# MicrobialDarkMatter/nanomotif

Measured on AMD Instinct MI355X. Metric: motif-sites scored/sec (1 Gbp synthetic metagenome), higher is better.
Workload: dtype u32 bit-planes / int64 counts

## Files before the change

nanomotif_amd/csrc/nmscan_device.h:

```cpp
#pragma once
#include "nmscan_internal.h"

namespace nmdetail {

__device__ __forceinline__ uint32_t alignbit(uint32_t hi, uint32_t lo, uint32_t sh) {
    return __builtin_amdgcn_alignbit(hi, lo, sh);
}

typedef const uint32_t __attribute__((address_space(4))) *cu32p;
typedef const uint8_t __attribute__((address_space(4))) *cu8p;

#ifndef NM_LIT_WAVES
#define NM_LIT_WAVES 4
#endif

template <int GN_, int GP_, bool COMPACT_, int NS_, bool LIT_, bool CF_, bool PC_ = false, bool CLS_ = false>
struct Variant {
    static constexpr int GN = GN_, GP = GP_, NS = NS_;
    static constexpr bool COMPACT = COMPACT_, LIT = LIT_, CF = CF_, PC = PC_;
    static constexpr bool CLS = CLS_;
    static_assert(!CLS || (GN == 1 && GP == 1 && COMPACT && NS == 1 && !LIT && !CF), "class planes: narrow compact heavy variants only");
    static constexpr int NW = T_WORDS + GN + GP;
    static constexpr int NP = LIT ? 4 : 8;
    static constexpr int NST = COMPACT ? 2 : 4;
    static constexpr int PDW = (GN + GP) * NP;
};

template <class K>
struct RawChunk {
    uint32_t h[K::NW], l[K::NW], v[K::NW];
    uint32_t s[K::NS][K::NST][T_WORDS];
    bool need_v;

    __device__ __forceinline__ void load(const Planes &seq, const StatePlanes (&stp)[K::NS], uint32_t chunk, int lane) {
        constexpr int GN = K::GN, GP = K::GP;
        need_v = ((cu8p)seq.needs_v)[chunk] != 0;
        const size_t base = (size_t)chunk * CHUNK_WORDS + (size_t)lane * T_WORDS;
#pragma unroll
        for (int j = 0; j < K::NS; ++j) {
            const uint32_t *src[4] = {K::COMPACT ? stp[j].M : stp[j].MP, K::COMPACT ? stp[j].U : stp[j].UP, stp[j].MM, stp[j].UM};
#pragma unroll
            for (int i = 0; i < K::NST; ++i) {
                const uint4 q = *reinterpret_cast<const uint4 *>(src[i] + base);
                s[j][i][0] = q.x; s[j][i][1] = q.y; s[j][i][2] = q.z; s[j][i][3] = q.w;
            }
        }
        const uint4 h4 = *reinterpret_cast<const uint4 *>(seq.H + base);
        const uint4 l4 = *reinterpret_cast<const uint4 *>(seq.L + base);
        h[GN + 0] = h4.x; h[GN + 1] = h4.y; h[GN + 2] = h4.z; h[GN + 3] = h4.w;
        l[GN + 0] = l4.x; l[GN + 1] = l4.y; l[GN + 2] = l4.z; l[GN + 3] = l4.w;
#pragma unroll
        for (int j = 0; j < GN; ++j) { h[j] = seq.H[base - GN + j]; l[j] = seq.L[base - GN + j]; }
#pragma unroll
        for (int j = 0; j < GP; ++j) { h[GN + T_WORDS + j] = seq.H[base + T_WORDS + j]; l[GN + T_WORDS + j] = seq.L[base + T_WORDS + j]; }
        if (need_v) {
            const uint4 v4 = *reinterpret_cast<const uint4 *>(seq.V + base);
            v[GN + 0] = v4.x; v[GN + 1] = v4.y; v[GN + 2] = v4.z; v[GN + 3] = v4.w;
#pragma unroll
            for (int j = 0; j < GN; ++j) v[j] = seq.V[base - GN + j];
#pragma unroll
            for (int j = 0; j < GP; ++j) v[GN + T_WORDS + j] = seq.V[base + T_WORDS + j];
        } else if constexpr (!K::CLS) {
#pragma unroll
            for (int j = 0; j < K::NW; ++j) v[j] = 0xFFFFFFFFu;
        }
    }
};

template <class K>
struct Tile {
    uint32_t w[K::NP][K::NW];

    __device__ __forceinline__ void expand(const RawChunk<K> &r) {
#pragma unroll
        for (int j = 0; j < K::NW; ++j) {
            const uint32_t hh = r.h[j], ll = r.l[j], vv = r.v[j];
            w[0][j] = vv & ~hh & ~ll;
            w[1][j] = vv & ~hh & ll;
            w[2][j] = vv & hh & ll;
            w[3][j] = vv & hh & ~ll;
            if (!K::LIT) {
                w[4][j] = vv & (hh | ll);
                w[5][j] = vv & (hh | ~ll);
                w[6][j] = vv & ~(hh & ll);
                w[7][j] = vv & (~hh | ll);
            }
        }
    }
};

template <class K>
__device__ __forceinline__ void eval_masks(const uint32_t (&m)[K::PDW], const Tile<K> &tile, uint32_t (&acc)[T_WORDS]) {
#pragma unroll
    for (int g = 0; g < K::GN + K::GP; ++g) {
#pragma unroll
        for (int p = 0; p < K::NP; ++p) {
            uint32_t mm = m[g * K::NP + p];
            while (mm) {
                const uint32_t r = __builtin_ctz(mm);
                mm &= mm - 1;
#pragma unroll
                for (int t = 0; t < T_WORDS; ++t) acc[t] &= alignbit(tile.w[p][t + g + 1], tile.w[p][t + g], r);
            }
        }
    }
}

constexpr int comp_plane(int p) { return (p & 4) | (3 - (p & 3)); }

template <class K>
struct JointWalk {
    uint32_t accf[T_WORDS], accr[T_WORDS];

    template <int G>
    static constexpr bool r0_possible() { return G > 0 && !(K::COMPACT && G == K::GN); }

    template <int I, bool R0 = false>
    __device__ __forceinline__ void and_in(const Tile<K> &tile, uint32_t r) {
        constexpr int G = I / K::NP, P = I % K::NP, CP = comp_plane(P), GR = R0 ? 2 * K::GN - G : 2 * K::GN - 1 - G;
        const uint32_t rr = R0 ? 0u : 32u - r;
#pragma unroll
        for (int t = 0; t < T_WORDS; ++t) accf[t] &= alignbit(tile.w[P][t + G + 1], tile.w[P][t + G], r);
#pragma unroll
        for (int t = 0; t < T_WORDS; ++t) accr[t] &= alignbit(tile.w[CP][t + GR + 1], tile.w[CP][t + GR], rr);
    }
    template <int I = 0>
    __device__ __forceinline__ void walk(const uint32_t (&m)[K::PDW], const Tile<K> &tile, const uint32_t (&bf)[T_WORDS],
                                         const uint32_t (&br)[T_WORDS]) {
        if constexpr (I == 0) {
#pragma unroll
            for (int t = 0; t < T_WORDS; ++t) { accf[t] = bf[t]; accr[t] = br[t]; }
        }
        if constexpr (I < K::PDW) {
            uint32_t mm = m[I];
            if (r0_possible<I / K::NP>() && (mm & 1u)) {
                mm &= ~1u;
                and_in<I, true>(tile, 0u);
            }
            while (mm) {
                const uint32_t r = __builtin_ctz(mm);
                mm &= mm - 1;
                and_in<I>(tile, r);
            }
            walk<I + 1>(m, tile, bf, br);
        }
    }
};

constexpr int CLS_PROG_DW = 32, CLS_SUMMARY_DW = 8, CLS_WORDS_DW = 9, CLS_BASE_DW = 29;
constexpr int cls_plane(int p) { return p < 4 ? p : p < 8 ? p - 4 : 4 + (p - 8) / 2; }
constexpr bool cls_neg(int p) { return p >= 4 && (p < 8 || ((p - 8) & 1)); }
constexpr int cls_mirror(int p) { return p < 4 ? 3 - p : p < 8 ? 11 - p : (p == 10 || p == 11) ? p : (p ^ 1); }
constexpr int cls_dword(int g, int p) { return p < 4 ? 4 * g + p : CLS_WORDS_DW + 10 * g + (p - 4); }
constexpr int cls_word_of_set(uint32_t set) {
    return set == 1 ? 0 : set == 2 ? 1 : set == 4 ? 2 : set == 8 ? 3 :
           set == 14 ? 4 : set == 13 ? 5 : set == 11 ? 6 : set == 7 ? 7 :
           set == 12 ? 8 : set == 3 ? 9 : set == 6 ? 10 : set == 9 ? 11 : set == 10 ? 12 : 13 ;
}

template <class K, bool BV>
struct ClassTile {
    static constexpr bool HAS_V = BV;
    static constexpr int VP = 6;
    uint32_t w[7][K::NW];

    __device__ __forceinline__ void expand(const RawChunk<K> &r) {
#pragma unroll
        for (int j = 0; j < K::NW; ++j) {
            const uint32_t hh = r.h[j], ll = r.l[j];
            w[0][j] = BV ? r.v[j] & ~(hh | ll) : ~(hh | ll);
            w[1][j] = ll & ~hh;
            w[2][j] = hh & ll;
            w[3][j] = hh & ~ll;
            w[4][j] = hh;
            w[5][j] = ll;
            w[6][j] = BV ? r.v[j] : hh ^ ll;
        }
    }
};

template <class K, class TileT>
struct ClassWalk {
    uint32_t accf[T_WORDS], accr[T_WORDS];

    template <int G, int P>
    __device__ __forceinline__ void and_one(const TileT &tile, uint32_t (&acc)[T_WORDS], uint32_t r) {
        constexpr int PL = cls_plane(P);
#pragma unroll
        for (int t = 0; t < T_WORDS; ++t) {
            uint32_t s;
            if constexpr (TileT::HAS_V && PL == 6) s = alignbit(tile.w[4][t + G + 1], tile.w[4][t + G], r) ^ alignbit(tile.w[5][t + G + 1], tile.w[5][t + G], r);
            else s = alignbit(tile.w[PL][t + G + 1], tile.w[PL][t + G], r);
            if constexpr (!cls_neg(P)) acc[t] &= s;
            else if constexpr (!TileT::HAS_V) acc[t] &= ~s;
            else acc[t] = acc[t] & ~s & alignbit(tile.w[TileT::VP][t + G + 1], tile.w[TileT::VP][t + G], r);
        }
    }
    template <int G, int P, bool R0 = false>
    __device__ __forceinline__ void and_in(const TileT &tile, uint32_t r) {
        constexpr int GR = R0 ? 2 * K::GN - G : 2 * K::GN - 1 - G;
        and_one<G, P>(tile, accf, r);
        and_one<GR, cls_mirror(P)>(tile, accr, R0 ? 0u : 32u - r);
    }
    template <int G, int P>
    __device__ __forceinline__ void word(uint32_t mm, const TileT &tile) {
        if (JointWalk<K>::template r0_possible<G>() && (mm & 1u)) {
            mm &= ~1u;
            and_in<G, P, true>(tile, 0u);
        }
        while (mm) {
            const uint32_t r = __builtin_ctz(mm);
            mm &= mm - 1;
            and_in<G, P>(tile, r);
        }
    }
    template <int Q>
    __device__ __forceinline__ void quad(const uint32_t (&m)[CLS_PROG_DW], const TileT &tile) {
        if (m[CLS_SUMMARY_DW] & (0xFu << (4 * Q))) {
            word<(4 * Q + 0) / 10, 4 + (4 * Q + 0) % 10>(m[CLS_WORDS_DW + 4 * Q + 0], tile);
            word<(4 * Q + 1) / 10, 4 + (4 * Q + 1) % 10>(m[CLS_WORDS_DW + 4 * Q + 1], tile);
            word<(4 * Q + 2) / 10, 4 + (4 * Q + 2) % 10>(m[CLS_WORDS_DW + 4 * Q + 2], tile);
            word<(4 * Q + 3) / 10, 4 + (4 * Q + 3) % 10>(m[CLS_WORDS_DW + 4 * Q + 3], tile);
        }
    }
    __device__ __forceinline__ void walk(const uint32_t (&m)[CLS_PROG_DW], const TileT &tile, const uint32_t (&)[T_WORDS],
                                         const uint32_t (&)[T_WORDS]) {
        const uint32_t cm = m[CLS_BASE_DW];
#pragma unroll
        for (int t = 0; t < T_WORDS; ++t) {
            accf[t] = (cm & tile.w[1][t + K::GN]) | (~cm & tile.w[0][t + K::GN]);
            accr[t] = (cm & tile.w[2][t + K::GN]) | (~cm & tile.w[3][t + K::GN]);
        }
        word<0, 0>(m[0], tile); word<0, 1>(m[1], tile); word<0, 2>(m[2], tile); word<0, 3>(m[3], tile);
        word<1, 0>(m[4], tile); word<1, 1>(m[5], tile); word<1, 2>(m[6], tile); word<1, 3>(m[7], tile);
        if (m[CLS_SUMMARY_DW]) {
            quad<0>(m, tile); quad<1>(m, tile); quad<2>(m, tile); quad<3>(m, tile); quad<4>(m, tile);
        }
    }
};

template <class K>
__device__ __forceinline__ void eval_strand(cu32p prog, const Tile<K> &tile, uint32_t (&acc)[T_WORDS]) {
    uint32_t m[K::PDW];
#pragma unroll
    for (int i = 0; i < K::PDW; ++i) m[i] = prog[i];
    eval_masks<K>(m, tile, acc);
}

inline uint32_t comp_mask(uint32_t m) { return ((m & 1) << 3) | ((m & 2) << 1) | ((m & 4) >> 1) | ((m & 8) >> 3); }

constexpr int PROG6_DW = 96;
inline int compile_program(const uint8_t *masks, uint32_t len, uint32_t modpos, uint32_t *prog, int *reach_class) {
    if (len == 0 || len > NM_MAX_MOTIF_LEN) return fail(NM_ERANGE, "motif length %u outside 1..%d", len, NM_MAX_MOTIF_LEN);
    if (modpos >= len) return fail(NM_EINVAL, "mod_position %u outside motif of length %u", modpos, len);
    memset(prog, 0, PROG6_DW * sizeof(uint32_t));
    bool any = false;
    *reach_class = 0;
    for (uint32_t j = 0; j < len; ++j) {
        const uint32_t m = masks[j] & 15u;
        if (m == 0) return fail(NM_EINVAL, "empty base set at motif position %u", j);
        if (m == 15u) continue;
        any = true;
        for (int strand = 0; strand < 2; ++strand) {
            const int d = strand == 0 ? (int)j - (int)modpos : (int)modpos - (int)j;
            const uint32_t set = strand == 0 ? m : comp_mask(m);
            const int gi = (d >> 5) + 3;
            const uint32_t r = (uint32_t)d & 31u;
            if (gi < 0 || gi > 5) return fail(NM_ERANGE, "offset %d from the modified base is outside [-96, 95]", d);
            *reach_class = std::max(*reach_class, gi == 0 || gi == 5 ? 2 : gi == 1 || gi == 4 ? 1 : 0);
            uint32_t *row = prog + strand * 48 + gi * 8;
            if (__builtin_popcount(set) == 1) {
                row[__builtin_ctz(set)] |= 1u << r;
            } else {
                uint32_t missing = (~set) & 15u;
                while (missing) {
                    row[4 + __builtin_ctz(missing)] |= 1u << r;
                    missing &= missing - 1;
                }
            }
        }
    }
    if (!any) return fail(NM_EINVAL, "motif has no specified position");
    return NM_OK;
}

inline void slice_program(const uint32_t *full, int G, uint32_t *out) {
    for (int strand = 0; strand < 2; ++strand)
        memcpy(out + strand * 2 * G * 8, full + strand * 48 + (3 - G) * 8, (size_t)2 * G * 8 * sizeof(uint32_t));
}

__device__ __forceinline__ void compile_one(uint32_t k, const CandRec *__restrict__ rec, const uint8_t *__restrict__ masks,
                                            uint32_t *__restrict__ programs, int wide, int np, int fold_modpos, uint32_t prog_slot = 0xFFFFFFFFu) {
    const int groups = 2 + 2 * wide, g0 = 1 - wide;
    const int pdw = 2 * groups * np;
    uint32_t *prog = programs + (size_t)(prog_slot == 0xFFFFFFFFu ? k : prog_slot) * pdw;
    for (int i = 0; i < pdw; ++i) prog[i] = 0;
    const CandRec c = rec[k];
    const uint8_t *m = masks + c.mask_off;
    for (int j = 0; j < c.len; ++j) {
        const uint32_t set_f = m[j] & 15u;
        if (set_f == 15u || (fold_modpos && j == c.modpos)) continue;
        for (int strand = 0; strand < 2; ++strand) {
            const int d = strand == 0 ? j - (int)c.modpos : (int)c.modpos - j;
            const uint32_t set = strand == 0 ? set_f
                                             : (((set_f & 1) << 3) | ((set_f & 2) << 1) | ((set_f & 4) >> 1) | ((set_f & 8) >> 3));
            const int g = (d >> 5) + 2 - g0;
            const uint32_t bit = 1u << ((uint32_t)d & 31u);
            uint32_t *row = prog + (strand * groups + g) * np;
            if (__popc(set) == 1) {
                row[__ffs(set) - 1] |= bit;
            } else {
                uint32_t missing = (~set) & 15u;
                while (missing) {
                    row[4 + __ffs(missing) - 1] |= bit;
                    missing &= missing - 1;
                }
            }
        }
    }
}

__device__ __forceinline__ void compile_one_classes(uint32_t k, const CandRec *__restrict__ rec, const uint8_t *__restrict__ masks,
                                                    uint32_t *__restrict__ programs, uint32_t c_slots) {
    uint32_t *prog = programs + (size_t)k * CLS_PROG_DW;
    for (int i = 0; i < CLS_PROG_DW; ++i) prog[i] = 0;
    const CandRec c = rec[k];
    const uint8_t *m = masks + c.mask_off;
    prog[CLS_BASE_DW] = ((c_slots >> c.slot) & 1u) ? 0xFFFFFFFFu : 0u;
    for (int j = 0; j < c.len; ++j) {
        const uint32_t set = m[j] & 15u;
        if (set == 15u || j == c.modpos) continue;
        const int d = j - (int)c.modpos;
        const int g = (d >> 5) + 1;
        if (g < 0 || g > 1) continue;
        const int p = cls_word_of_set(set);
        prog[cls_dword(g, p)] |= 1u << ((uint32_t)d & 31u);
        if (p >= 4) prog[CLS_SUMMARY_DW] |= 1u << (10 * g + p - 4);
    }
}

__device__ __forceinline__ void common_one(uint32_t g, uint4 *__restrict__ range, uint32_t *programs, uint32_t *commons, uint32_t pdw,
                                           uint32_t n_prog, uint32_t max_group) {
    uint4 r = range[g];
    r.z = 0xFFFFFFFFu;
    r.w = 0;
    if (r.y >= 2 && r.y <= max_group) {
        uint32_t *common = commons + (size_t)g * pdw;
        uint32_t any = 0;
        for (uint32_t i = 0; i < pdw; ++i) {
            uint32_t c = programs[(size_t)r.x * pdw + i];
            for (uint32_t k = 1; k < r.y; ++k) c &= programs[(size_t)(r.x + k) * pdw + i];
            common[i] = c;
            any |= c;
        }
        if (any) {
            bool single = true;
            const uint32_t sdw = pdw / 2;
            for (uint32_t k = 0; k < r.y; ++k) {
                uint32_t *prog = programs + (size_t)(r.x + k) * pdw;
                for (uint32_t i = 0; i < pdw; ++i) prog[i] &= ~common[i];
                for (uint32_t st = 0; st < 2; ++st) {
                    uint32_t bits = 0;
                    for (uint32_t i = 0; i < sdw; ++i) bits += __popc(prog[st * sdw + i]);
                    if (bits > 1) single = false;
                }
            }
            if (single) {
                for (uint32_t k = 0; k < r.y; ++k) {
                    uint32_t *prog = programs + (size_t)(r.x + k) * pdw;
                    uint32_t desc[2];
                    for (uint32_t st = 0; st < 2; ++st) {
                        desc[st] = sdw << 5;
                        for (uint32_t i = 0; i < sdw; ++i)
                            if (prog[st * sdw + i]) desc[st] = (i << 5) | (uint32_t)(__ffs(prog[st * sdw + i]) - 1);
                    }
                    prog[0] = desc[0];
                    prog[1] = desc[1];
                }
                r.w = 1;
            }
            r.z = n_prog + g;
        }
    }
    range[g] = r;
}


}

#ifdef NM_SCORE_KERNEL_SOURCE

namespace nmdetail {

struct ScoreArgs {
    Planes seq;
    StatePlanes st[NM_MAX_MOD_SLOTS];
    const uint4 *segments;
    uint32_t n_segments;
    uint32_t split_log2;
    uint32_t pieces_per_run, j_big, fine_log2;
    uint32_t n_bins;
    const uint4 *cand_range;
    const uint32_t *programs;
    const uint32_t *orig_index;
    unsigned long long *out;
    const uint32_t *chunk_rank;
    const uint64_t *row_base;
    uint32_t active_slot[NM_MAX_MOD_SLOTS];
    uint32_t slot_is_c[NM_MAX_MOD_SLOTS];
};

void launch_score_classes(const ScoreArgs &a, uint32_t gx, uint32_t gy, bool per_contig, hipStream_t s);

}

namespace {

using namespace nmdetail;

template <class K, int I = 0>
__device__ __forceinline__ void apply_single(uint32_t idx, uint32_t r, const Tile<K> &tile, const uint32_t (&base)[T_WORDS],
                                             uint32_t (&acc)[T_WORDS]) {
    if constexpr (I < K::PDW) {
        if (idx == I) {
            constexpr int g = I / K::NP, p = I % K::NP;
#pragma unroll
            for (int t = 0; t < T_WORDS; ++t) acc[t] = base[t] & alignbit(tile.w[p][t + g + 1], tile.w[p][t + g], r);
        } else {
            apply_single<K, I + 1>(idx, r, tile, base, acc);
        }
    } else {
#pragma unroll
        for (int t = 0; t < T_WORDS; ++t) acc[t] = base[t];
    }
}

template <class K>
__device__ __forceinline__ void emit_counts(const ScoreArgs &a, uint32_t n_mod, uint32_t n_non, uint32_t k0, uint32_t k,
                                            uint32_t *lds_acc, uint32_t lds_row0, int lane, uint32_t contig_rank) {
    if (K::PC) {
#pragma unroll
        for (int o = 32; o; o >>= 1) {
            n_mod += __shfl_xor(n_mod, o);
            n_non += __shfl_xor(n_non, o);
        }
        if (lane == 0 && (n_mod | n_non)) {
            unsigned long long *row = a.out + (a.row_base[k0 + k] + contig_rank) * 2;
            if (n_mod) atomicAdd(row, (unsigned long long)n_mod);
            if (n_non) atomicAdd(row + 1, (unsigned long long)n_non);
        }
        return;
    }
    atomicAdd(&lds_acc[((k * K::NS + lds_row0) * 2 + 0) * 64 + lane], n_mod);
    atomicAdd(&lds_acc[((k * K::NS + lds_row0) * 2 + 1) * 64 + lane], n_non);
}

template <class K, int CAN, class TileT>
__device__ __forceinline__ void score_heavy(const ScoreArgs &a, const TileT &tile, const uint32_t (&sw)[K::NST][T_WORDS],
                                            uint32_t k0, uint32_t nb, uint32_t *lds_acc, uint32_t lds_row0, int lane,
                                            uint32_t contig_rank) {
    constexpr int PF = CAN == 0 ? 0 : 1;
    constexpr int PR = CAN == 0 ? 3 : 2;
    uint32_t basef[T_WORDS], baser[T_WORDS];
#pragma unroll
    for (int t = 0; t < T_WORDS; ++t) {
        basef[t] = K::COMPACT ? tile.w[PF][t + K::GN] : 0xFFFFFFFFu;
        baser[t] = K::COMPACT ? tile.w[PR][t + K::GN] : 0xFFFFFFFFu;
    }
    constexpr int MDW = K::CLS ? CLS_PROG_DW : K::PDW;
    static_assert(!K::CLS || CLS_PROG_DW == 2 * K::PDW, "a class program takes the room of both halves of a plain one");
    std::conditional_t<K::CLS, ClassWalk<K, TileT>, JointWalk<K>> jw;
    for (uint32_t k = 0; k < nb; ++k) {
        cu32p prog = (cu32p)(a.programs + (size_t)(k0 + k) * (2 * K::PDW));
        uint32_t m[MDW];
        if constexpr (K::CLS) {
            typedef uint32_t u32x16 __attribute__((ext_vector_type(16)));
            typedef const u32x16 __attribute__((address_space(4))) *cu32x16p;
            const u32x16 lo = ((cu32x16p)prog)[0], hi = ((cu32x16p)prog)[1];
#pragma unroll
            for (int i = 0; i < 16; ++i) { m[i] = lo[i]; m[16 + i] = hi[i]; }
        } else {
#pragma unroll
            for (int i = 0; i < MDW; ++i) m[i] = prog[i];
        }
        jw.walk(m, tile, basef, baser);
        uint32_t n_mod = 0, n_non = 0;
#pragma unroll
        for (int t = 0; t < T_WORDS; ++t) {
            if (K::COMPACT) {
                const uint32_t sites = jw.accf[t] | jw.accr[t];
                n_mod += __popc(sites & sw[0][t]);
                n_non += __popc(sites & sw[1][t]);
            } else {
                n_mod += __popc(jw.accf[t] & sw[0][t]) + __popc(jw.accr[t] & sw[K::COMPACT ? 0 : 2][t]);
                n_non += __popc(jw.accf[t] & sw[1][t]) + __popc(jw.accr[t] & sw[K::COMPACT ? 1 : 3][t]);
            }
        }
        emit_counts<K>(a, n_mod, n_non, k0, k, lds_acc, lds_row0, lane, contig_rank);
    }
}

template <class K, int CAN, class TileT>
__device__ __forceinline__ void score_candidates(const ScoreArgs &a, const TileT &tile, const uint32_t (&sw)[K::NST][T_WORDS],
                                                 uint32_t k0, uint32_t nb, uint32_t common, bool siblings, uint32_t *lds_acc,
                                                 uint32_t lds_row0, int lane, uint32_t contig_rank = 0) {
    if constexpr (!K::CF) {
        score_heavy<K, CAN>(a, tile, sw, k0, nb, lds_acc, lds_row0, lane, contig_rank);
        return;
    } else {
    constexpr int PF = CAN == 0 ? 0 : 1;
    constexpr int PR = CAN == 0 ? 3 : 2;
    uint32_t basef[T_WORDS], baser[T_WORDS];
#pragma unroll
    for (int t = 0; t < T_WORDS; ++t) {
        basef[t] = K::COMPACT ? tile.w[PF][t + K::GN] : 0xFFFFFFFFu;
        baser[t] = K::COMPACT ? tile.w[PR][t + K::GN] : 0xFFFFFFFFu;
    }
    if (common != 0xFFFFFFFFu) {
        cu32p prog = (cu32p)(a.programs + (size_t)common * (2 * K::PDW));
        eval_strand<K>(prog, tile, basef);
        eval_strand<K>(prog + K::PDW, tile, baser);
    }
    uint32_t mf[K::PDW], mr[K::PDW];
    if (!siblings) {
        cu32p prog = (cu32p)(a.programs + (size_t)k0 * (2 * K::PDW));
#pragma unroll
        for (int i = 0; i < K::PDW; ++i) mf[i] = prog[i];
    }
    for (uint32_t k = 0; k < nb; ++k) {
        cu32p prog = (cu32p)(a.programs + (size_t)(k0 + k) * (2 * K::PDW));
        uint32_t accf[T_WORDS], accr[T_WORDS];
        if (siblings) {
            const uint32_t df = prog[0], dr = prog[1];
            apply_single<K>(df >> 5, df & 31u, tile, basef, accf);
            apply_single<K>(dr >> 5, dr & 31u, tile, baser, accr);
        } else {
#pragma unroll
            for (int i = 0; i < K::PDW; ++i) mr[i] = prog[K::PDW + i];
#pragma unroll
            for (int t = 0; t < T_WORDS; ++t) accf[t] = basef[t];
            eval_masks<K>(mf, tile, accf);
            cu32p next = (cu32p)(a.programs + (size_t)(k0 + min(k + 1, nb - 1)) * (2 * K::PDW));
#pragma unroll
            for (int i = 0; i < K::PDW; ++i) mf[i] = next[i];
#pragma unroll
            for (int t = 0; t < T_WORDS; ++t) accr[t] = baser[t];
            eval_masks<K>(mr, tile, accr);
        }
        uint32_t n_mod = 0, n_non = 0;
#pragma unroll
        for (int t = 0; t < T_WORDS; ++t) {
            if (K::COMPACT) {
                const uint32_t sites = accf[t] | accr[t];
                n_mod += __popc(sites & sw[0][t]);
                n_non += __popc(sites & sw[1][t]);
            } else {
                n_mod += __popc(accf[t] & sw[0][t]) + __popc(accr[t] & sw[K::COMPACT ? 0 : 2][t]);
                n_non += __popc(accf[t] & sw[1][t]) + __popc(accr[t] & sw[K::COMPACT ? 1 : 3][t]);
            }
        }
        emit_counts<K>(a, n_mod, n_non, k0, k, lds_acc, lds_row0, lane, contig_rank);
    }
    }
}

template <class T>
struct TileTag { using type = T; };

template <class K>
__device__ __forceinline__ void score_piece(const ScoreArgs &a, const uint4 sg, const StatePlanes (&stp)[K::NS], const bool (&is_c)[K::NS],
                                            uint32_t *lds_acc, const int lane, const uint32_t wave) {
    constexpr int NS = K::NS;
    constexpr uint32_t H = BMAX / NS;
    constexpr bool EARLY = K::CF && K::LIT;
    RawChunk<K> first;
    if (EARLY && wave < sg.y) first.load(a.seq, stp, sg.x + wave, lane);
    uint4 range[NS];
    uint32_t most = 0;
#pragma unroll
    for (int j = 0; j < NS; ++j) {
        const uint32_t slot_i = NS == 1 ? blockIdx.y : (uint32_t)j;
        range[j] = a.cand_range[(size_t)slot_i * a.n_bins + sg.z];
        range[j].x = __builtin_amdgcn_readfirstlane(range[j].x);
        range[j].y = __builtin_amdgcn_readfirstlane(range[j].y);
        range[j].z = __builtin_amdgcn_readfirstlane(range[j].z);
        range[j].w = __builtin_amdgcn_readfirstlane(range[j].w);
        most = max(most, range[j].y);
    }
    if (most == 0) return;

    auto score_tile = [&](auto tile_tag, const RawChunk<K> &cur, uint32_t pass0, uint32_t chunk) {
        typename decltype(tile_tag)::type tile;
        tile.expand(cur);
        const uint32_t rank = K::PC ? ((cu32p)a.chunk_rank)[chunk] : 0u;
        auto one_slot = [&](auto jc) {
            constexpr int j = decltype(jc)::value;
            if (range[j].y <= pass0) return;
            const uint32_t nbj = min(H, range[j].y - pass0);
            if constexpr (K::CLS)
                score_candidates<K, 0>(a, tile, cur.s[j], range[j].x + pass0, nbj, range[j].z, range[j].w != 0, lds_acc, j, lane, rank);
            else if (K::COMPACT && is_c[j])
                score_candidates<K, 1>(a, tile, cur.s[j], range[j].x + pass0, nbj, range[j].z, range[j].w != 0, lds_acc, j, lane, rank);
            else
                score_candidates<K, 0>(a, tile, cur.s[j], range[j].x + pass0, nbj, range[j].z, range[j].w != 0, lds_acc, j, lane, rank);
        };
        one_slot(std::integral_constant<int, 0>{});
        if constexpr (NS > 1) one_slot(std::integral_constant<int, 1>{});
        static_assert(NS <= 2, "slot fusion is written for one or two slots");
    };
    auto score_chunk = [&](const RawChunk<K> &cur, uint32_t pass0, uint32_t chunk) {
        if constexpr (K::CLS) {
            if (cur.need_v) score_tile(TileTag<ClassTile<K, true>>{}, cur, pass0, chunk);
            else score_tile(TileTag<ClassTile<K, false>>{}, cur, pass0, chunk);
        } else {
            score_tile(TileTag<Tile<K>>{}, cur, pass0, chunk);
        }
    };
    auto clear_rows = [&](uint32_t rows_hi) {
        if (K::PC) return;
        for (uint32_t i = threadIdx.x; i < rows_hi * 128; i += 256) lds_acc[i] = 0;
        __syncthreads();
    };
    auto flush_rows = [&](uint32_t rows_hi, uint32_t pass0) {
        if (K::PC) return;
        __syncthreads();
        for (uint32_t idx = threadIdx.x; idx < rows_hi * 8; idx += 256) {
            const uint32_t i = idx >> 2, q = idx & 3;
            const uint32_t j = (i >> 1) % NS, k = (i >> 1) / NS;
            uint32_t s = 0;
#pragma unroll 4
            for (int jj = 0; jj < 16; ++jj) s += lds_acc[i * 64 + q * 16 + jj];
            s += __shfl_xor(s, 1);
            s += __shfl_xor(s, 2);
            if (q == 0 && s) {
                uint4 rj = range[0];
#pragma unroll
                for (int t = 1; t < NS; ++t)
                    if (j == (uint32_t)t) rj = range[t];
                if (pass0 + k < rj.y) {
                    const uint32_t orig = a.orig_index[rj.x + pass0 + k];
                    atomicAdd(a.out + (size_t)orig * 2 + (i & 1), (unsigned long long)s);
                }
            }
        }
        __syncthreads();
    };
    uint32_t pass0 = 0;
    if (EARLY) {
        const uint32_t rows_hi = NS * min(H, most);
        clear_rows(rows_hi);
        if (wave < sg.y) score_chunk(first, 0, sg.x + wave);
        for (uint32_t ck = wave + 4; ck < sg.y; ck += 4) {
            RawChunk<K> cur;
            cur.load(a.seq, stp, sg.x + ck, lane);
            score_chunk(cur, 0, sg.x + ck);
        }
        flush_rows(rows_hi, 0);
        pass0 = H;
    }
    for (; pass0 < most; pass0 += H) {
        const uint32_t rows_hi = NS * min(H, most - pass0);
        clear_rows(rows_hi);
        for (uint32_t ck = wave; ck < sg.y; ck += 4) {
            RawChunk<K> cur;
            cur.load(a.seq, stp, sg.x + ck, lane);
            score_chunk(cur, pass0, sg.x + ck);
        }
        flush_rows(rows_hi, pass0);
    }
}

#define NM_SCORE_BOUNDS __launch_bounds__(256, (K::GN + K::GP > 2 ? 2 : (K::LIT ? NM_LIT_WAVES : (K::CLS ? 6 : 4))))

#define NM_SLOT_SETUP                                                                                               \
    const int lane = threadIdx.x & 63;                                                                              \
    const uint32_t wave = __builtin_amdgcn_readfirstlane(threadIdx.x >> 6);  \
    StatePlanes stp[K::NS];                                                                                         \
    bool is_c[K::NS];                                                                                               \
    _Pragma("unroll") for (int j = 0; j < K::NS; ++j) {                                                             \
        const uint32_t slot = a.active_slot[K::NS == 1 ? blockIdx.y : (uint32_t)j];                                 \
        stp[j] = a.st[slot];                                                                                        \
        is_c[j] = a.slot_is_c[slot] != 0;                                                                           \
    }

template <class K>
__global__ NM_SCORE_BOUNDS void score_kernel(ScoreArgs a) {
    __shared__ uint32_t lds_acc[BMAX * 2 * 64];
    const uint32_t lanes_x = K::CF ? 1u : 8u;
    const uint32_t x = K::CF ? 0u : blockIdx.x % 8, j = K::CF ? blockIdx.x : blockIdx.x / 8;
    uint32_t piece, sub = 0, n_sub = 1;
    if (j < a.j_big) piece = x * a.pieces_per_run + j;
    else {
        const uint32_t k = j - a.j_big;
        piece = x * a.pieces_per_run + a.j_big + (k >> a.fine_log2);
        sub = k & ((1u << a.fine_log2) - 1);
        n_sub = 1u << a.fine_log2;
        if (a.j_big + (k >> a.fine_log2) >= a.pieces_per_run) return;
    }
    (void)lanes_x;
    const uint32_t seg = piece >> a.split_log2;
    if (seg >= a.n_segments) return;
    uint4 sg = a.segments[seg];
    sg.x = __builtin_amdgcn_readfirstlane(sg.x);
    sg.y = __builtin_amdgcn_readfirstlane(sg.y);
    sg.z = __builtin_amdgcn_readfirstlane(sg.z);
    if (a.split_log2) {
        const uint32_t len = (sg.y + (1u << a.split_log2) - 1) >> a.split_log2;
        const uint32_t at = (piece & ((1u << a.split_log2) - 1)) * len;
        if (at >= sg.y) return;
        sg.x += at;
        sg.y = min(len, sg.y - at);
    }
    if (n_sub > 1) {
        const uint32_t len = (sg.y + n_sub - 1) / n_sub;
        const uint32_t at = sub * len;
        if (at >= sg.y) return;
        sg.x += at;
        sg.y = min(len, sg.y - at);
    }
    NM_SLOT_SETUP
    score_piece<K>(a, sg, stp, is_c, lds_acc, lane, wave);
}

}

#ifdef NM_SCORE_CLASSES_UNIT
namespace nmdetail {

void launch_score_classes(const ScoreArgs &a, uint32_t gx, uint32_t gy, bool per_contig, hipStream_t s) {
    if (per_contig) hipLaunchKernelGGL((score_kernel<Variant<1, 1, true, 1, false, false, true, true>>), dim3(gx, gy), dim3(256), 0, s, a);
    else hipLaunchKernelGGL((score_kernel<Variant<1, 1, true, 1, false, false, false, true>>), dim3(gx, gy), dim3(256), 0, s, a);
}

}
#endif

#endif
```

Measured before the change: 93890 billion.

## Fold C-slot base swap into class tile expansion and use swizzle reductions

For class-plane variants, C-slot candidates now have their base sets remapped A<->C, G<->T when programs are compiled. The tile expansion applies the swap once per tile by XORing the low bit-plane with a per-block mask, so the walk no longer blends two planes under the base mask for every candidate. The per-contig count reduction in the class path also switches from shuffle-xor to ds_swizzle plus a readlane. Static asserts check the swap mapping, and the change relies on every slot in a block sharing the same C-ness, taken from is_c[0].

```diff
diff --git a/nanomotif_amd/csrc/nmscan_device.h b/nanomotif_amd/csrc/nmscan_device.h
--- a/nanomotif_amd/csrc/nmscan_device.h
+++ b/nanomotif_amd/csrc/nmscan_device.h
@@ -157,6 +157,22 @@
            set == 14 ? 4 : set == 13 ? 5 : set == 11 ? 6 : set == 7 ? 7 :
            set == 12 ? 8 : set == 3 ? 9 : set == 6 ? 10 : set == 9 ? 11 : set == 10 ? 12 : 13 ;
 }
+constexpr uint32_t cls_swap_set(uint32_t set) { return ((set & 5u) << 1) | ((set & 10u) >> 1); }
+constexpr int cls_swap_word(int p) { return p < 8 ? (p ^ 1) : p < 10 ? p : (p ^ 1); }
+constexpr uint32_t cls_comp_set(uint32_t set) { return ((set & 1u) << 3) | ((set & 2u) << 1) | ((set & 4u) >> 1) | ((set & 8u) >> 3); }
+constexpr bool cls_swap_ok() {
+    for (uint32_t set = 1; set < 15; ++set) {
+        const int p = cls_word_of_set(set), q = cls_word_of_set(cls_swap_set(set));
+        if (cls_swap_set(cls_swap_set(set)) != set) return false;
+        if (q != cls_swap_word(p)) return false;
+        if (cls_mirror(p) != cls_word_of_set(cls_comp_set(set))) return false;
+        if (cls_mirror(q) != cls_swap_word(cls_mirror(p))) return false;
+    }
+    return true;
+}
+static_assert(cls_swap_ok(), "A<->C, G<->T swap of a base set: class word and mirror, all 14 sets");
+static_assert(cls_word_of_set(cls_swap_set(2)) == 0 && cls_word_of_set(cls_swap_set(4)) == 3,
+              "a C slot's canonical base is plane 0 of its tile, the complement plane 3");
 
 template <class K, bool BV>
 struct ClassTile {
@@ -164,10 +180,13 @@
     static constexpr int VP = 6;
     uint32_t w[7][K::NW];
 
-    __device__ __forceinline__ void expand(const RawChunk<K> &r) {
+    __device__ __forceinline__ void expand(const RawChunk<K> &r, const uint32_t cm) {
 #pragma unroll
         for (int j = 0; j < K::NW; ++j) {
-            const uint32_t hh = r.h[j], ll = r.l[j];
+            const uint32_t hh = r.h[j];
+            uint32_t ll = r.l[j] ^ cm;
+            asm("" : "+v"(ll));
+            if (BV) ll &= r.v[j];
             w[0][j] = BV ? r.v[j] & ~(hh | ll) : ~(hh | ll);
             w[1][j] = ll & ~hh;
             w[2][j] = hh & ll;
@@ -225,11 +244,10 @@
     }
     __device__ __forceinline__ void walk(const uint32_t (&m)[CLS_PROG_DW], const TileT &tile, const uint32_t (&)[T_WORDS],
                                          const uint32_t (&)[T_WORDS]) {
-        const uint32_t cm = m[CLS_BASE_DW];
 #pragma unroll
         for (int t = 0; t < T_WORDS; ++t) {
-            accf[t] = (cm & tile.w[1][t + K::GN]) | (~cm & tile.w[0][t + K::GN]);
-            accr[t] = (cm & tile.w[2][t + K::GN]) | (~cm & tile.w[3][t + K::GN]);
+            accf[t] = tile.w[0][t + K::GN];
+            accr[t] = tile.w[3][t + K::GN];
         }
         word<0, 0>(m[0], tile); word<0, 1>(m[1], tile); word<0, 2>(m[2], tile); word<0, 3>(m[3], tile);
         word<1, 0>(m[4], tile); word<1, 1>(m[5], tile); word<1, 2>(m[6], tile); word<1, 3>(m[7], tile);
@@ -326,10 +344,12 @@
     for (int i = 0; i < CLS_PROG_DW; ++i) prog[i] = 0;
     const CandRec c = rec[k];
     const uint8_t *m = masks + c.mask_off;
-    prog[CLS_BASE_DW] = ((c_slots >> c.slot) & 1u) ? 0xFFFFFFFFu : 0u;
+    const bool swap = ((c_slots >> c.slot) & 1u) != 0;
+    prog[CLS_BASE_DW] = swap ? 0xFFFFFFFFu : 0u;
     for (int j = 0; j < c.len; ++j) {
-        const uint32_t set = m[j] & 15u;
+        uint32_t set = m[j] & 15u;
         if (set == 15u || j == c.modpos) continue;
+        if (swap) set = cls_swap_set(set);
         const int d = j - (int)c.modpos;
         const int g = (d >> 5) + 1;
         if (g < 0 || g > 1) continue;
@@ -439,10 +459,20 @@
 __device__ __forceinline__ void emit_counts(const ScoreArgs &a, uint32_t n_mod, uint32_t n_non, uint32_t k0, uint32_t k,
                                             uint32_t *lds_acc, uint32_t lds_row0, int lane, uint32_t contig_rank) {
     if (K::PC) {
-#pragma unroll
-        for (int o = 32; o; o >>= 1) {
-            n_mod += __shfl_xor(n_mod, o);
-            n_non += __shfl_xor(n_non, o);
+        if constexpr (K::CLS) {
+#define NM_SWZ_ADD(o)                                                                         \
+            n_mod += (uint32_t)__builtin_amdgcn_ds_swizzle((int)n_mod, ((o) << 10) | 0x1f); \
+            n_non += (uint32_t)__builtin_amdgcn_ds_swizzle((int)n_non, ((o) << 10) | 0x1f);
+            NM_SWZ_ADD(16) NM_SWZ_ADD(8) NM_SWZ_ADD(4) NM_SWZ_ADD(2) NM_SWZ_ADD(1)
+#undef NM_SWZ_ADD
+            n_mod += (uint32_t)__builtin_amdgcn_readlane((int)n_mod, 32);
+            n_non += (uint32_t)__builtin_amdgcn_readlane((int)n_non, 32);
+        } else {
+#pragma unroll
+            for (int o = 32; o; o >>= 1) {
+                n_mod += __shfl_xor(n_mod, o);
+                n_non += __shfl_xor(n_non, o);
+            }
         }
         if (lane == 0 && (n_mod | n_non)) {
             unsigned long long *row = a.out + (a.row_base[k0 + k] + contig_rank) * 2;
@@ -588,10 +618,12 @@
         most = max(most, range[j].y);
     }
     if (most == 0) return;
+    const uint32_t cm = K::CLS ? __builtin_amdgcn_readfirstlane(is_c[0] ? 0xFFFFFFFFu : 0u) : 0u;
 
     auto score_tile = [&](auto tile_tag, const RawChunk<K> &cur, uint32_t pass0, uint32_t chunk) {
         typename decltype(tile_tag)::type tile;
-        tile.expand(cur);
+        if constexpr (K::CLS) tile.expand(cur, cm);
+        else tile.expand(cur);
         const uint32_t rank = K::PC ? ((cu32p)a.chunk_rank)[chunk] : 0u;
         auto one_slot = [&](auto jc) {
             constexpr int j = decltype(jc)::value;
```

Result: faster. 97800 billion, median of 6 (+4.2%).
